# mastbaum/sxmc

Measured on AMD Instinct MI355X. Metric: NLL evals/sec (10^8 samples, 3 obs, 12 signals) + experiments/sec at 1/2/4/8 GPUs, higher is better.
Workload: dtype f64 exact; f32-on-u16-codes filter decides the unambiguous samples

## Files before the change

sxmc_amd/csrc/fill_kernels.inc.h:

```cpp
#pragma once

#include "sxmc_device_types.h"

#pragma clang fp contract(off)

#ifndef SXMC_MEASURE
#define SXMC_MEASURE 0
#endif

namespace sxfill {

__device__ __forceinline__ constexpr unsigned sx_dbg(unsigned dbg_arg) { return SXMC_MEASURE ? dbg_arg : 0u; }

template <int N>
struct IntC {
  static constexpr int value = N;
  constexpr operator int() const { return N; }
};
template <unsigned long... I>
struct ISeq {};
template <int N, unsigned long... I>
struct MakeISeq : MakeISeq<N - 1, (unsigned long)(N - 1), I...> {};
template <unsigned long... I>
struct MakeISeq<0, I...> {
  typedef ISeq<I...> type;
// ... 479 lines not shown
#pragma unroll 4
      for (unsigned b = tid; b < B; b += nthreads) {
        const unsigned c = hist[b];
        if (c != 0u) __hip_atomic_fetch_add(&gbins[b], c, __ATOMIC_RELAXED, __HIP_MEMORY_SCOPE_AGENT);
      }
      if (si + 1u < seg_end) {
        __syncthreads();
        for (unsigned b = tid; b < B; b += nthreads) hist[b] = 0u;
      }
    }
    if (tid == 0) {
      const unsigned c = *s_norm;
      if (c != 0u) __hip_atomic_fetch_add(to_global(d.norm), c, __ATOMIC_RELAXED, __HIP_MEMORY_SCOPE_AGENT);
      *s_norm = 0u;
    }
    __syncthreads();
    lds_clean = true;
  }
}

constexpr int kPreOrdered = kFormOrdered;
constexpr int kPreBoxed = kFormBoxed;
constexpr unsigned kOrdMixed = 0xFFFFFFFEu, kOrdSkip = 0xFFFFFFFFu;
typedef float vfloat2 __attribute__((ext_vector_type(2)));

template <unsigned OPC>
__device__ __forceinline__ void apply_ordered_scalar(double& x, const double* c) {
  constexpr int type = (int)(OPC & 15u);
  static_assert(sx_op_npars(OPC) == 1 && (type == SXMC_SYST_SHIFT || type == SXMC_SYST_SCALE || type == SXMC_SYST_CTSCALE),
                "not a monotone systematic");
  const double pc = 0.0 + c[0] * 1.0;
  if constexpr (type == SXMC_SYST_SHIFT) x = x + pc;
  if constexpr (type == SXMC_SYST_SCALE) x = x * (1 + pc);
  if constexpr (type == SXMC_SYST_CTSCALE) x = 1 + (x - 1) * (1 + pc);
}
template <int ORD, unsigned... OPS, unsigned long... I>
__device__ __forceinline__ void run_ordered_scalar(double& x, const double* c, StaticProg<OPS...>, ISeq<I...>) {
  ([&] {
    if constexpr ((int)((OPS >> 4) & 15u) == ORD) apply_ordered_scalar<OPS>(x, c + sx_prog_cstart<OPS...>((int)I));
  }(), ...);
}
template <int NSLOT, int ORD, bool WANT, unsigned... OPS, unsigned long... I>
__device__ __forceinline__ void run_static_part(double (&f)[NSLOT][SXMC_VEC], const double* c, StaticProg<OPS...>,
                                                ISeq<I...>) {
  ([&] {
    if constexpr (((int)((OPS >> 4) & 15u) == ORD) == WANT) apply_static<NSLOT, OPS>(f, c + sx_prog_cstart<OPS...>((int)I));
// ... 1300 lines not shown
  fin = fin && (__builtin_fabs(xl) < __builtin_inf()) && (__builtin_fabs(xh) < __builtin_inf());
}
template <int BX, int XT, unsigned... OPS, unsigned long... I>
__device__ __forceinline__ void run_box_interval(double& xl, double& xh, double tl, double th, bool& fin, const double* c,
                                                 StaticProg<OPS...>, ISeq<I...>) {
  ([&] {
    if constexpr ((int)((OPS >> 4) & 15u) == BX) apply_box_interval<OPS, XT>(xl, xh, tl, th, fin, c + sx_prog_cstart<OPS...>((int)I));
  }(), ...);
}
template <int BX, int XT, unsigned... OPS>
constexpr bool prog_is_boxable(StaticProg<OPS...>) {
  return (true && ... &&
          (sx_op_npars(OPS) == 1 && (int)((OPS >> 4) & 15u) != XT &&
           ((int)(OPS & 15u) != SXMC_SYST_RESOLUTION_SCALE ||
            ((int)((OPS >> 4) & 15u) == BX && (int)((OPS >> 8) & 15u) == XT))));
}

#ifndef SXMC_BOX_DRAIN
#define SXMC_BOX_DRAIN 2
#endif
#ifndef SXMC_BOX_GQ
#define SXMC_BOX_GQ 0
#endif
#ifndef SXMC_BOX_PREFETCH
#define SXMC_BOX_PREFETCH 0
#endif
template <int NOBS, int NSLOT, typename PROG>
__device__ __forceinline__ void fill_boxed_body(const SxSignalDesc* __restrict__ descs, const SxSegment* __restrict__ segs,
                                                const unsigned* __restrict__ blk_off, unsigned layout, unsigned dbg_arg) {
  const unsigned dbg = sx_dbg(dbg_arg);
  static_assert(!PROG::dynamic && NOBS == 1 && NSLOT == 3, "one streamed observable, one truth field, the boxed observable");
  constexpr int BX = 2, XT = 1;
  static_assert(prog_is_boxable<BX, XT>(PROG{}), "not a program the boxed form can run");
  constexpr int NC = PROG::ncoef > 0 ? PROG::ncoef : 1;
#ifndef SXMC_BOX_RING
#define SXMC_BOX_RING 8
#endif
  constexpr int kRing = SXMC_BOX_RING;
  constexpr int kDrain = SXMC_BOX_DRAIN;
  static_assert(64 % kRing == 0, "a block of 64 units is a whole number of rounds of the ring");
  typedef typename MakeISeq<PROG::n>::type Seq;
  extern __shared__ unsigned lds[];
  const unsigned tid = threadIdx.x;
  const unsigned nthreads = blockDim.x;
  const unsigned lane = tid & (kWave - 1);
  unsigned* s_norm = lds;
// ... 76 lines not shown
      g = g + form[0].a[0] * (d.qbase[0] + 0.5 * d.qstep[0]);
      g = g * sc;
      const double mu = sum_abs * 65536.0 + __builtin_fabs(g) + (double)nbk + 0.25;
      const double epsq = 0.5 * sum_abs * (1.0 + 0x1p-19);
      const double eps = epsq + mu * 0x1p-21 + (form[0].mag + __builtin_fabs(lo)) * sc * 0x1p-44;
      const bool ok = eps < 0.125;
      double e = eps * 1.01, slack = 0x1p-23;
#if SXMC_MEASURE
      {
        const unsigned fr = (dbg >> 8) & 0xFFu, ft = (dbg >> 16) & 0xFFu;
        const double rs = fr ? (double)(fr - 1u) / 64.0 : 1.0, ts = ft ? (double)(ft - 1u) / 64.0 : 1.0;
        e = (epsq + rs * (e - epsq)) * ts;
        slack = slack * rs * ts;
      }
#endif
      af = uniform_f((float)alpha);
      gf = uniform_f((float)(g + e));
      thr = uniform_f((float)(2.0 * e + slack));
      use_q = use_q && (uniform_i(ok ? 1 : 0) != 0);
    }

    unsigned vcnt = 0u;
    unsigned nrow = 0u, ngran = 0u;

    unsigned gword = kOrdSkip, greal = 0u;
    vfloat4 bx_next;
    unsigned pre_next;
    auto meta_load = [&](unsigned it) {
      unsigned vg = vwave32 + (it + lane) * step32;
      vg = vg <= vlast32 ? vg : vlast32;
      bx_next = boxes[vg >> 6];
      pre_next = precol[vg >> 6];
    };
    auto granule_meta = [&](unsigned it) {
      unsigned vg = vwave32 + (it + lane) * step32;
      const bool live = vg <= vlast32;
      vg = live ? vg : vlast32;
      if constexpr (!SXMC_BOX_PREFETCH) meta_load(it);
      const vfloat4 bx = bx_next;
      const unsigned pre = pre_next;
      if constexpr (SXMC_BOX_PREFETCH) meta_load(it + 64u);
      double xl = (double)bx.x, xh = (double)bx.y;
      const double tl = (double)bx.z, th = (double)bx.w;
      bool fin = (__builtin_fabs(xl) < __builtin_inf()) && (__builtin_fabs(xh) < __builtin_inf()) &&
                 (__builtin_fabs(tl) < __builtin_inf()) && (__builtin_fabs(th) < __builtin_inf());
      run_box_interval<BX, XT>(xl, xh, tl, th, fin, craw, PROG{}, Seq{});
      const int i0 = (int)((xl - olo) * osc), i1 = (int)((xh - olo) * osc);
      const int e0 = !(xl >= olo) ? -1 : (!(xl < ohi) ? 0x7FFFFFFF : i0);
      const int e1 = !(xh >= olo) ? -1 : (!(xh < ohi) ? 0x7FFFFFFF : i1);
      const unsigned off = (pre & 0xFFFFFFu) + (unsigned)e0 * (unsigned)ost;
      const unsigned h = fdiv(off, inv_out), rem = off - h * s_out;
      const bool canon = off < (1u << 22) && rem < s_in && (h + 1u) * s_out <= B;
      const bool mixed = !use_q || !fin || e0 != e1 || !canon;
      const bool skip = fin && e0 == e1 && (e0 < 0 || e0 == 0x7FFFFFFF);
      gword = !live ? kOrdSkip : skip ? kOrdSkip : mixed ? kOrdMixed : h * s_in + rem;
      greal = off;
    };

    auto push_granule = [&](unsigned it) {
      if (lane == 0) qgran[2u * ngran] = vwave32 + it * step32;
      ngran += 1u;
    };
    auto push_rows = [&](unsigned rare, unsigned v, unsigned real_off) -> bool {
      unsigned long long mask[SXMC_VEC];
      unsigned total = 0u;
#pragma unroll
      for (int q = 0; q < SXMC_VEC; q++) {
        mask[q] = __builtin_amdgcn_ballot_w64(((rare >> q) & 1u) != 0u);
        total += (unsigned)__builtin_popcountll(mask[q]);
      }
      if (nrow + total > rq_cap) return false;
#pragma unroll
      for (int q = 0; q < SXMC_VEC; q++) {
        if (mask[q] == 0ull) continue;
        const unsigned below = __builtin_amdgcn_mbcnt_hi((unsigned)(mask[q] >> 32),
                                                         __builtin_amdgcn_mbcnt_lo((unsigned)mask[q], 0u));
        if ((rare >> q) & 1u) {
          const unsigned pos = nrow + below;
          qrows[2u * pos] = v * SXMC_VEC + (unsigned)q;
          qrows[2u * pos + 1u] = real_off;
        }
        nrow += (unsigned)__builtin_popcountll(mask[q]);
      }
      return true;
    };

    const int oS4 = (int)(4u * oSp);
    const int oclamp = (dbg & 4u) ? -1 : (int)nbk;
    auto coarse_unit = [&](const vuint2g& w, unsigned it, unsigned v, unsigned word0) {
      int base4 = (int)(4u * (4u + myrep + word0) + 4u * oSp);
      asm volatile("" : "+v"(base4));
      const float c0 = (float)(w.x & 0xFFFFu), c1 = (float)(w.x >> 16), c2 = (float)(w.y & 0xFFFFu), c3 = (float)(w.y >> 16);
      const vfloat2 a2 = {af, af}, g2 = {gf, gf};
      const vfloat2 u01 = __builtin_elementwise_fma(a2, vfloat2{c0, c1}, g2);
      const vfloat2 u23 = __builtin_elementwise_fma(a2, vfloat2{c2, c3}, g2);
      const float us[SXMC_VEC] = {u01.x, u01.y, u23.x, u23.y};
      int addr[SXMC_VEC];
      bool amb[SXMC_VEC];
#pragma unroll
      for (int q = 0; q < SXMC_VEC; q++) {
        const float u = us[q];
        amb[q] = !(__builtin_amdgcn_fractf(u) >= thr);
        int idx;
        asm("v_cvt_flr_i32_f32 %0, %1" : "=v"(idx) : "v"(u));
        int ie;
        asm("v_med3_i32 %0, %1, -1, %2" : "=v"(ie) : "v"(amb[q] ? -1 : idx), "s"(oclamp));
        addr[q] = mad24(ie, oS4, base4);
      }
      const float cmax = __builtin_fmaxf(__builtin_fmaxf(c0, c1), __builtin_fmaxf(c2, c3));
      const bool special = cmax >= (float)SXMC_QCODE_EXACT;
      const bool anyamb = (amb[0] | amb[1]) | (amb[2] | amb[3]);
      if (__builtin_amdgcn_ballot_w64(anyamb || special) != 0ull) {
        const float cs[SXMC_VEC] = {c0, c1, c2, c3};
        unsigned rare = 0u;
#pragma unroll
        for (int q = 0; q < SXMC_VEC; q++) {
          rare |= amb[q] ? (1u << q) : 0u;
          if (cs[q] >= (float)SXMC_QCODE_EXACT) {
            addr[q] = base4 - oS4;
            rare = cs[q] >= (float)SXMC_QCODE_NEVER ? (rare & ~(1u << q)) : (rare | (1u << q));
          }
        }
        const unsigned real_off = (unsigned)__builtin_amdgcn_readlane((int)greal, (int)(it & 63u));
        if (!push_rows(rare, v, real_off)) {
          push_granule(it);
          return;
        }
      }
      if (dbg & 32u) {
        vcnt += (unsigned)(addr[0] ^ addr[1] ^ addr[2] ^ addr[3]) == 12345u ? 1u : 0u;
        return;
      }
#pragma unroll
      for (int q = 0; q < SXMC_VEC; q++) {
        unsigned* wp = reinterpret_cast<unsigned*>(reinterpret_cast<char*>(lds) + addr[q]);
        __hip_atomic_fetch_add(wp, 1u, __ATOMIC_RELAXED, __HIP_MEMORY_SCOPE_WORKGROUP);
      }
    };

    auto count_exact = [&](bool ind, int bin) {
      vcnt += (ind && !((unsigned)bin < B)) ? 1u : 0u;
      if (ind && ((unsigned)bin < B)) {
        __hip_atomic_fetch_add(&hist[myrep + hist_word((unsigned)bin)], 1u, __ATOMIC_RELAXED, __HIP_MEMORY_SCOPE_WORKGROUP);
      }
    };
    auto drain = [&]() {
      if (dbg & 16u) nrow = ngran = 0u;
      vfloat4 rawf[kDrain][NSLOT];
      unsigned prew[kDrain];
      auto load_granule = [&](int s, unsigned g) {
        const unsigned vw = (unsigned)uniform_i((int)qgran[2u * g]);
        const unsigned vc = vw + lane < vlast32 ? vw + lane : vlast32;
#pragma unroll
        for (int k = 0; k < NSLOT; k++) rawf[s][k] = __builtin_nontemporal_load(&col[k][vc]);
        prew[s] = precol[vc >> 6];
      };
      unsigned row = 0u, w1 = 0u;
      float rowf = 0.0f;
// ... 64 lines not shown
      rq[slot] = __builtin_nontemporal_load((gptr<const vuint2g>)((gptr<const char>)qcol + (unsigned long long)o));
      __builtin_amdgcn_sched_barrier(0);
    };
    const unsigned climit = (unsigned)uniform_i((int)oS);
    {
      unsigned it = 0u;
      if constexpr (SXMC_BOX_PREFETCH) meta_load(0u);
#pragma unroll
      for (int i = 0; i < kRing; i++) issue(i, (unsigned)i);
      while (it < niter32) {
        if ((it & 63u) == 0u) granule_meta(it);
        const unsigned block_end = niter32 < (it | 63u) + 1u ? niter32 : (it | 63u) + 1u;
        bool full = false;
        while (it < block_end && !full) {
#pragma unroll
          for (int i = 0; i < kRing; i++) {
#pragma unroll
            for (int e = 0; e < 2; e++) asm volatile("" : "+v"(rq[i][e]));
            const unsigned iu = it + (unsigned)i;
            if (iu < block_end) {
              const unsigned word0 = (unsigned)__builtin_amdgcn_readlane((int)gword, (int)(iu & 63u));
              if (dbg & 1u) {
                vcnt += (rq[i].x == 12345u && word0 == 77u) ? 1u : 0u;
              } else if (word0 < climit) coarse_unit(rq[i], iu, vfirst32 + iu * step32, word0);
              else if (word0 == kOrdMixed) push_granule(iu);
            }
            issue(i, iu + (unsigned)kRing);
          }
          it = block_end - it < (unsigned)kRing ? block_end : it + (unsigned)kRing;
          full = ngran + (unsigned)kRing > gq_drain;
        }
        if (full) {
          drain();
          __builtin_amdgcn_s_waitcnt(0);
        }
      }
    }
    drain();

    {
      unsigned t = vcnt;
#pragma unroll
      for (int off = kWave / 2; off > 0; off >>= 1) t += __shfl_down(t, off, kWave);
      if (lane == 0 && t != 0u) __hip_atomic_fetch_add(&s_norm[0], t, __ATOMIC_RELAXED, __HIP_MEMORY_SCOPE_WORKGROUP);
    }
    __syncthreads();
    {
      gptr<unsigned> gbins = to_global(d.bins);
      const bool more = si + 1u < seg_end;
      const unsigned nwords = nbk * oSp;
      const float invSp = 1.0f / (float)oSp;
      unsigned total = 0u;
#pragma unroll 4
      for (unsigned w = tid; w < nwords; w += nthreads) {
        const unsigned idx = fdiv(w, invSp), r = w - idx * oSp;
        unsigned n = 0u;
        for (unsigned rep = 0; rep < R; rep++) n += hist[rep * rstride + oSp + w];
        if (r < oS) {
          total += n;
          const unsigned h = fdiv(r, inv_in);
          if (n != 0u) {
            __hip_atomic_fetch_add(&gbins[h * s_out + idx * s_in + (r - h * s_in)], n, __ATOMIC_RELAXED, __HIP_MEMORY_SCOPE_AGENT);
          }
        }
      }
#pragma unroll
      for (int off = kWave / 2; off > 0; off >>= 1) total += __shfl_down(total, off, kWave);
      if (lane == 0 && total != 0u) __hip_atomic_fetch_add(&s_norm[0], total, __ATOMIC_RELAXED, __HIP_MEMORY_SCOPE_WORKGROUP);
      __syncthreads();
      if (more) {
        for (unsigned b = 4u * tid; b < cstride; b += 4u * nthreads) {
          *reinterpret_cast<vuint4g*>(&hist[b]) = vuint4g{0u, 0u, 0u, 0u};
        }
      }
      if (tid == 0) {
        const unsigned n = s_norm[0];
        if (n != 0u) __hip_atomic_fetch_add(to_global(d.norm), n, __ATOMIC_RELAXED, __HIP_MEMORY_SCOPE_AGENT);
        s_norm[0] = 0u;
      }
    }
    __syncthreads();
    lds_clean = true;
  }
}

template <int NOBS, int NSLOT, bool LDS_HIST, typename PROG, int PREW>
__global__ __launch_bounds__(1024) void fill_kernel(const SxSignalDesc* __restrict__ descs,
                                                    const SxSegment* __restrict__ segs,
                                                    const unsigned* __restrict__ blk_off, unsigned hist_words,
                                                    unsigned dbg) {
  fill_body<NOBS, NSLOT, LDS_HIST, PROG, PREW>(descs, segs, blk_off, hist_words, dbg);
}

template <int NOBS, int NSLOT, typename PROG>
__global__ __launch_bounds__(1024) void fill_sparse_kernel(const SxSignalDesc* __restrict__ descs,
                                                           const SxSegment* __restrict__ segs,
                                                           const unsigned* __restrict__ blk_off, unsigned smax,
                                                           unsigned dbg) {
  fill_sparse_body<NOBS, NSLOT, PROG>(descs, segs, blk_off, smax, dbg);
}

#ifndef SXMC_ORDERED_BOUND
// ... 22 lines not shown
```

sxmc_amd/csrc/layout_kernels.hip:

```cpp
#include "nll_device.h"
#include "sxmc_host.h"

#include <hipcub/hipcub.hpp>

#include <cmath>
#include <cstring>
#include <limits>

#pragma clang fp contract(off)

namespace {

struct KeyPlan {
  unsigned mask;
  unsigned outside;
  unsigned radix[SXMC_MAX_NFIELDS];
};

__global__ __launch_bounds__(256) void bucket_key_kernel(const SxSignalDesc* __restrict__ dp, KeyPlan plan,
                                                         const unsigned* __restrict__ rows_in,
                                                         unsigned* __restrict__ keys, unsigned* __restrict__ rows) {
  const SxSignalDesc& d = *dp;
  const unsigned long long n = d.nsamples;
  const unsigned long long step = (unsigned long long)gridDim.x * blockDim.x;
// ... 199 lines not shown
                                                             unsigned long long n, unsigned short* __restrict__ qcol,
                                                             unsigned* __restrict__ tally) {
  const unsigned long long step = (unsigned long long)gridDim.x * blockDim.x;
  unsigned nexact = 0u, nnever = 0u;
  for (unsigned long long i = (unsigned long long)blockIdx.x * blockDim.x + threadIdx.x; i < n; i += step) {
    const double x = (double)col[i];
    unsigned code;
    if (!(fabs(x) < __builtin_inf())) {
      code = SXMC_QCODE_NEVER;
      nnever++;
    } else {
      const double t = (x - base) / qstep;
      bool exact = !(t >= 0.0 && t < (double)(SXMC_QCODE_MAX + 1u));
      const unsigned q = exact ? 0u : (unsigned)t;
      const double centre = base + ((double)q + 0.5) * qstep;
      if (!(fabs(x - centre) <= 0.5 * qstep * (1.0 + 0x1p-20))) exact = true;
      code = exact ? SXMC_QCODE_EXACT : q;
      nexact += exact ? 1u : 0u;
    }
    qcol[i] = (unsigned short)code;
  }
  if (nexact) atomicAdd(&tally[0], nexact);
  if (nnever) atomicAdd(&tally[1], nnever);
}

struct SampleGeom {
  int nobs;
  int has_cuts;
  int nbins[3];
  double lower[3], upper[3], width[3];
  double scale[3];
  float bottom[3], top[3];
  float cut_lo[3], cut_hi[3];
};

__device__ __forceinline__ int sample_side(float xf, unsigned idx, double lower, double upper, double scale) {
  const double x = (double)xf;
  if (!(x >= lower)) return -1;
  if (!(x < upper)) return 1;
  const long long j = (long long)((x - lower) * scale);
  return j < (long long)idx ? -1 : j > (long long)idx ? 1 : 0;
}

__device__ __forceinline__ float sample_float(double xd, unsigned idx, const SampleGeom& g, int k) {
  const float x0 = (float)xd;
  float xf = x0;
// ... 194 lines not shown
}

hipError_t sx_column_codes16(const float* col, double base, double step, unsigned long long n, unsigned short* qcol,
                             unsigned long long* tally, hipStream_t s) {
  sxhost::DeviceBuffer<unsigned> tmp;
  hipError_t e = (hipError_t)tmp.alloc(2);
  if (e != hipSuccess) return e;
  unsigned* const d = tmp.get();
  e = hipMemsetAsync(d, 0, sizeof(unsigned) * 2, s);
  if (e == hipSuccess && n) {
    hipLaunchKernelGGL(column_codes16_kernel, dim3(grid_for(n, 16384)), dim3(256), 0, s, col, base, step, n, qcol, d);
    e = hipGetLastError();
  }
  unsigned h[2] = {0u, 0u};
  if (e == hipSuccess) e = hipMemcpyAsync(h, d, sizeof h, hipMemcpyDeviceToHost, s);
  hipError_t e2 = hipStreamSynchronize(s);
  if (tally) {
    tally[0] = h[0];
    tally[1] = h[1];
  }
  return e != hipSuccess ? e : e2;
}

hipError_t sx_hist_cdf(const unsigned* d_bins, unsigned* d_cdf, int nbins_total, hipStream_t s) {
  size_t temp_bytes = 0;
  hipError_t e = hipcub::DeviceScan::InclusiveSum(nullptr, temp_bytes, d_bins, d_cdf, nbins_total, s);
  if (e != hipSuccess) return e;
  sxhost::DeviceBuffer<void> temp;
  e = (hipError_t)temp.alloc(temp_bytes ? temp_bytes : 16);
  if (e != hipSuccess) return e;
  e = hipcub::DeviceScan::InclusiveSum(temp.get(), temp_bytes, d_bins, d_cdf, nbins_total, s);
  hipError_t e2 = hipStreamSynchronize(s);
  return e != hipSuccess ? e : e2;
}

hipError_t sx_inclusive_sum_u32(const unsigned* d_in, unsigned* d_out, int n, void* temp, size_t& temp_bytes,
                                hipStream_t s) {
  return hipcub::DeviceScan::InclusiveSum(temp, temp_bytes, d_in, d_out, n, s);
}

hipError_t sx_random_sample(const unsigned* d_cdf, int nbins_total, int nobs, const int* nbins, const double* lower,
                            const double* upper, const double* scale, const float* cut_lo, const float* cut_hi,
                            unsigned long long seed, unsigned long long n, float dataset, float* d_out,
                            unsigned* d_exhausted, hipStream_t s) {
  if (n == 0) return hipSuccess;
  SampleGeom g{};
// ... 21 lines not shown
```

sxmc_amd/csrc/sxmc_device.h:

```cpp
#pragma once

#include <hip/hip_runtime.h>
#include <stdint.h>

#include <string>

#include "../../include/sxmc_hip.h"

#include "step_end_plan.h"
#include "sxmc_device_types.h"

struct SxStepArgs {
  size_t nsignals, nsources;
  const double* means;
  const double* sigmas;
  sxmc_rng_state* rng;
  double* nll_current;
  double* nll_proposed;
  double* v_current;
  double* v_proposed;
  int* accepted;
  int* counter;
  float* jump_buffer;
  int nparameters;
// ... 124 lines not shown
hipError_t sx_launch_fill(const SxLaunchShape& shape, const SxSignalDesc* d_descs, const SxSegment* d_segs,
                          const unsigned* d_blk_off, hipStream_t s);
hipError_t sx_launch_fill_sparse_runs(const SxLaunchShape& shape, const SxSignalDesc* d_descs, const SxSegment* d_segs,
                                      const unsigned* d_blk_off, hipStream_t s);
bool sx_fill_has_specialization(int nobs, int nslot);
int sx_fill_find_program(int form, int nobs, int nslot, int nops, const unsigned* ops);
bool sx_fill_supports(int prog, int form, int lds_hist, int sparse_runs);
bool sx_fill_weighted_supports(int prog, int lds_hist);
hipError_t sx_launch_prebin(const SxSignalDesc* d_desc, unsigned long long npad, unsigned mask, int width, void* out,
                            hipStream_t s);
hipError_t sx_bucket_keys(const SxSignalDesc* d_desc, unsigned long long nsamples, unsigned mask, const unsigned* radix,
                          unsigned outside, const unsigned* d_rows_in, unsigned* d_keys, unsigned* d_rows,
                          hipStream_t s);
hipError_t sx_order_keys(const float* d_col, unsigned long long nsamples, unsigned* d_keys, unsigned* d_rows,
                         hipStream_t s);
hipError_t sx_bucket_edges(const float* d_col, const unsigned* d_valid, unsigned long long ngranules, float* d_edges,
                           hipStream_t s);
hipError_t sx_box_keys(const float* d_colx, const float* d_colt, unsigned long long nsamples, int pass, int nstrata,
                       const unsigned* bounds, unsigned* d_keys, unsigned* d_rows, hipStream_t s);
hipError_t sx_bucket_boxes(const float* d_colx, const float* d_colt, const unsigned* d_valid, unsigned long long ngranules,
                           float* d_boxes, hipStream_t s);
hipError_t sx_column_codes16(const float* col, double base, double step, unsigned long long n, unsigned short* qcol,
                             unsigned long long* tally, hipStream_t s);
hipError_t sx_bucket_sort(const unsigned* keys_in, unsigned* keys_out, const unsigned* rows_in, unsigned* rows_out,
                          unsigned long long n, int bits, hipStream_t s);
hipError_t sx_bucket_first(const unsigned* sorted_keys, unsigned long long n, unsigned* d_first, hipStream_t s);
hipError_t sx_bucket_gather(const float* cols, unsigned long long pitch, int ncols, const int* col_list,
                            const unsigned* sorted_rows, const unsigned* d_src, const unsigned* d_valid,
                            unsigned long long ngranules, float* out, unsigned long long out_pitch, hipStream_t s);
hipError_t sx_column_minmax(const float* cols, unsigned long long pitch, int ncols, unsigned long long n, float* out,
                            hipStream_t s);
hipError_t sx_column_codes(const float* cols, unsigned long long pitch, int nslots, const double* base, const double* step,
                           unsigned long long n, unsigned* qcol, unsigned long long* tally, hipStream_t s);
hipError_t sx_hist_cdf(const unsigned* d_bins, unsigned* d_cdf, int nbins_total, hipStream_t s);
hipError_t sx_random_sample(const unsigned* d_cdf, int nbins_total, int nobs, const int* nbins, const double* lower,
                            const double* upper, const double* scale, const float* cut_lo, const float* cut_hi,
                            unsigned long long seed, unsigned long long n, float dataset, float* d_out,
                            unsigned* d_exhausted, hipStream_t s);
hipError_t sx_hist_project(const unsigned* d_bins, unsigned long long total, unsigned stride, unsigned nb,
                           unsigned long long* d_out, unsigned max_blocks, hipStream_t s);
hipError_t sx_launch_eval_pdf(const SxSignalDesc* d_descs, int nsig, unsigned long long max_points,
                              hipStream_t s);
template <typename W>
hipError_t sx_launch_eval_nll(const SxSignalDesc* d_descs, int nsig, unsigned long long npoints,
                              const W* weight, const double* pars, const double* nexpected, const unsigned* n_mc,
                              const short* source_id, const unsigned* norms, double* sums,
// ... 91 lines not shown
```

sxmc_amd/csrc/sxmc_group.cpp:

```cpp
#include "sxmc_host.h"

using namespace sxhost;

namespace sxhost {
std::atomic<int> g_stepping_groups{0};

int proposal_factor_check(const double* factor, int nparameters, size_t nsignals) {
  if (factor && (nparameters > 256 || nsignals > 256)) {
    return fail(SXMC_ERR_SHAPE, "a proposal factor needs the staged step end: at most 256 parameters and 256 signals");
  }
  return SXMC_OK;
}

SxStepArgs sx_step_args(const sxmc_step_args& p, size_t nsignals, const double* factor) {
  SxStepArgs a;
  a.factor = factor;
  a.nsignals = nsignals;
  a.nsources = p.nsources;
  a.means = p.d_means;
  a.sigmas = p.d_sigmas;
  a.rng = p.d_rng;
  a.nll_current = p.d_nll_current;
  a.nll_proposed = p.d_nll_proposed;
  a.v_current = p.d_v_current;
// ... 960 lines not shown
}

static void algorithmic_bytes(const sxmc_group* g, const LaunchPlan& plan, double* fill_read, double* hist, double* event) {
  double fr = 0, hb = 0, ev = 0;
  for (size_t i = 0; i < g->members.size(); i++) {
    const sxmc_hist* h = g->members[i];
    const SxSignalDesc& d = g->h_descs[i];
    int pre_w = 0, pre_dims = 0;
    bool codes = false;
    for (const LaunchClass& c : plan.classes) {
      for (int idx : c.member_idx) {
        if (idx == (int)i && c.shape.form != kFormRows) {
          pre_w = sx_form_pre_bytes(c.shape.form);
          for (int k = 0; k < d.nobs; k++) pre_dims += (c.pre_mask >> k) & 1u;
        }
        if (idx == (int)i) codes = c.codes;
      }
    }
    if (const SampleStore::Bucketed* bk = i < plan.member_bucket.size() ? plan.member_bucket[i] : nullptr) {
      const bool ord = bk->sort && bk->sort->ordered >= 0;
      const bool box = ord && bk->sort->box_truth >= 0;
      const double row_bytes = (codes && bk->d_qcol) ? (bk->q16 ? 2.0 : 4.0 * (double)((bk->nq + 1) / 2))
                                                     : 4.0 * (double)(bk->fields.size() - (ord ? 1 : 0));
      fr += (double)bk->nkept * row_bytes + ((box ? 16.0 : ord ? 8.0 : 0.0) + (bk->runs > 1 ? 8.0 : 4.0)) * (double)bk->ngranules;
    } else {
      fr += (double)h->nsamples * (4.0 * (d.nslot - pre_dims) + pre_w + (h->mult ? 4.0 : 0.0));
    }
    if (h->total_nbins <= kLdsMaxBins) {
      hb += 4.0 * (double)h->total_nbins;
    } else if (g->sparse_ready && g->cfg_sparse) {
      hb += 2.0 * 4.0 * (double)std::max(h->ntargets, 1);
    } else {
      hb += 2.0 * 4.0 * (double)h->total_nbins;
    }
    ev += 16.0 * (double)d.npoints;
  }
  *fill_read = fr;
  *hist = hb;
  *event = ev;
}

int sxmc_group_algorithmic_bytes(sxmc_group_t g, double* fill_read, double* hist, double* event) {
  SX_REQUIRE(g && fill_read && hist && event, "null argument");
  int rc = group_refresh(g);
  if (rc) return rc;
  algorithmic_bytes(g, active_plan(g), fill_read, hist, event);
  return SXMC_OK;
// ... 4 lines not shown
```

sxmc_amd/csrc/sxmc_launch_plan.cpp:

```cpp
#include "sxmc_host.h"

using namespace sxhost;

namespace sxhost {

using sxplan::apportion_workgroups;

template <typename T>
hipError_t upload(const std::vector<T>& v, DeviceBuffer<T>& d, size_t room = 0) {
  const hipError_t e = (hipError_t)d.alloc(std::max(v.size(), room));
  return (e != hipSuccess || v.empty()) ? e : hipMemcpy(d.get(), v.data(), sizeof(T) * v.size(), hipMemcpyHostToDevice);
}

void member_slots(const sxmc_hist* h, std::vector<int>& slot_col) {
  slot_col.clear();
  for (int k = 0; k < h->nobs; k++) slot_col.push_back(k);
  std::vector<int> extra;
  for (const HostSyst& s : h->systs) {
    if (s.obs >= h->nobs) extra.push_back(s.obs);
    if (s.type == SXMC_SYST_RESOLUTION_SCALE && s.extra_field >= h->nobs) extra.push_back(s.extra_field);
  }
  std::sort(extra.begin(), extra.end());
  extra.erase(std::unique(extra.begin(), extra.end()), extra.end());
  for (int c : extra) slot_col.push_back(c);
// ... 223 lines not shown
  b->runs = runs;
  b->sort = bs;
  sxplan::BucketedLayout lay;
  sxplan::bucketed_layout(bs->lsrc, bs->lvalid, bs->lwhich, bs->keys, bs->key_pre, bs->nkeys_total, runs, pack_rows, lay);
  const size_t P = lay.P, A = lay.A;
  const std::vector<unsigned>&psrc = lay.psrc, &pvalid = lay.pvalid, &ppre = lay.ppre, &pkp = lay.pkp;
  b->ngranules = P;
  b->nkept = bs->nkept;
  b->pitch = std::max<size_t>(64, P * 256);
  DeviceBuffer<unsigned> dsrc, dvalid;
  SX_BUF(b->d_cols.alloc(b->pitch * fields.size()));
  SX_BUF(b->d_gpre.alloc(A));
  SX_BUF(b->d_gkp.alloc(2 * A));
  SX_HIP(hipMemcpy(b->d_gpre.get(), ppre.data(), sizeof(unsigned) * A, hipMemcpyHostToDevice));
  SX_HIP(hipMemcpy(b->d_gkp.get(), pkp.data(), sizeof(unsigned) * 2 * A, hipMemcpyHostToDevice));
  SX_BUF(dsrc.alloc(A ? A : 4));
  SX_BUF(dvalid.alloc(A ? A : 4));
  SX_HIP(hipMemcpy(dsrc.get(), psrc.data(), A * 4, hipMemcpyHostToDevice));
  SX_HIP(hipMemcpy(dvalid.get(), pvalid.data(), A * 4, hipMemcpyHostToDevice));
  SX_HIP(sx_bucket_gather(st.d_cols.get(), h->pitch, (int)fields.size(), fields.data(), bs->d_rows.get(), dsrc.get(),
                          dvalid.get(), P, b->d_cols.get(), b->pitch, nullptr));
  if (bs->ordered >= 0 && bs->box_truth >= 0) {
    SX_REQUIRE(fields.size() >= 2, "a boxed layout streams its observable and the truth field");
    SX_BUF(b->d_gbox.alloc(4 * A));
    SX_HIP(hipMemset(b->d_gbox.get(), 0xFF, sizeof(float) * 4 * A));
    SX_HIP(sx_bucket_boxes(b->d_cols.get() + (fields.size() - 1) * b->pitch, b->d_cols.get() + (fields.size() - 2) * b->pitch,
                           dvalid.get(), P, b->d_gbox.get(), nullptr));
    {
      std::vector<float> hb(4 * P);
      if (P) SX_HIP(hipMemcpy(hb.data(), b->d_gbox.get(), sizeof(float) * 4 * P, hipMemcpyDeviceToHost));
      std::vector<double> ex, et;
      for (size_t p = 0; p < P; p++) {
        const float x0 = hb[4 * p], x1 = hb[4 * p + 1], t0 = hb[4 * p + 2], t1 = hb[4 * p + 3];
        if (!(std::isfinite(x0) && std::isfinite(x1) && std::isfinite(t0) && std::isfinite(t1))) continue;
        ex.push_back((double)x1 - (double)x0);
        et.push_back((double)t1 - (double)t0);
      }
      auto trimmed = [](std::vector<double>& v) {
        if (v.empty()) return 0.0;
        std::sort(v.begin(), v.end());
        const size_t keep = std::max<size_t>(1, v.size() * 9 / 10);
        double sum = 0;
        for (size_t i = 0; i < keep; i++) sum += v[i];
        return sum / (double)keep;
      };
      b->box_dx = trimmed(ex);
      b->box_dt = trimmed(et);
    }
// ... 37 lines not shown
    b->qbase[m] = cw.base[(size_t)m];
    b->qstep[m] = cw.step[(size_t)m];
  }
  double ambiguous = 0;
  for (int m = 0; m < nq && m < cd.nobs; m++) ambiguous += (double)cd.nbins[m] * cw.step[(size_t)m] / (cd.upper[m] - cd.lower[m]);
  static const bool gate_lifted = [] {
    const char* e = measure_env("SXMC_CODES_GATE");
    return e && e[0] == '1';
  }();
  if (!(ambiguous <= 2e-3) && !gate_lifted) return SXMC_OK;
  if (b->d_qcol.alloc(boxed ? b->pitch / 2 : b->pitch * (size_t)((nq + 1) / 2)) != 0) {
    (void)hipGetLastError();
    return SXMC_OK;
  }
  unsigned long long tally[2] = {0, 0};
  b->q16 = boxed;
  hipError_t e = boxed ? sx_column_codes16(b->d_cols.get(), b->qbase[0], b->qstep[0], n, reinterpret_cast<unsigned short*>(b->d_qcol.get()),
                                           tally, nullptr)
                       : sx_column_codes(b->d_cols.get(), b->pitch, nq, b->qbase, b->qstep, n, b->d_qcol.get(), tally, nullptr);
  if (e != hipSuccess || (double)tally[0] > 0.02 * (double)std::max<size_t>(b->nkept, 1)) {
    b->d_qcol.reset();
    if (e != hipSuccess) return fail(SXMC_ERR_HIP, std::string("codes of a bucketed table: ") + hipGetErrorString(e));
    return SXMC_OK;
  }
  b->nq = nq;
  b->q_exact_rows = tally[0];
  b->q_never_rows = tally[1];
  return SXMC_OK;
}


int build_bucket_tables(sxmc_hist* h, const SampleStore::BucketSort* bs) {
  if (h->btab_valid && h->btab_mask == bs->mask && h->btab_points_version == h->points_version) return SXMC_OK;
  reset_bucket_tables(h);
  sxplan::BucketTables bt;
  sxplan::bucket_tables(bs->nkeys_total, bs->mask, bs->radix, h->nbins.data(), h->stride.data(), h->nobs, h->targets, bt);
  const std::vector<unsigned>&dir = bt.dir, &tkeys = bt.tkeys, &tslot = bt.tslot;
  SX_HIP(upload(dir, h->d_bdir));
  SX_HIP(upload(tkeys, h->d_btkeys, 4));
  SX_HIP(upload(tslot, h->d_btslot, 4));
  h->btab_mask = bs->mask;
  h->btab_points_version = h->points_version;
  h->btab_valid = true;
  return SXMC_OK;
}

// ... 692 lines not shown
```

sxmc_amd/csrc/sxmc_rtc.cpp:

```cpp
#include <hip/hip_runtime.h>
#include <hip/hip_ext.h>
#include <hip/hiprtc.h>

#include <map>
#include <mutex>
#include <string>
#include <vector>

#include "rtc_sources.h"
#include "sxmc_device.h"

namespace {

std::mutex g_mutex;
std::map<std::string, hipFunction_t> g_cache;
std::map<std::string, std::string> g_failed;

std::string join(const char* const* pieces) {
  std::string s;
  for (int i = 0; pieces[i]; i++) s += pieces[i];
  return s;
}

std::string signature(bool chains, int bound, bool dbg = true) {
// ... 29 lines not shown
           ", 1>(one, segs, blk_off, w, dbg);\n}\n";
  }
  if (k.nchain > 1) {
    return s + signature(true, 1024, false) + "  fill_multi_body<" + shape + prog + ", " + std::to_string(k.form) + ", " +
           std::to_string(k.nchain) + ">(chains, segs, blk_off, w);\n}\n";
  }
  if (k.sparse_runs) {
    return s + signature(false, 1024) + "  fill_sparse_body<" + shape + prog + ">(descs, segs, blk_off, w, dbg);\n}\n";
  }
  return s + signature(false, 1024) + "  fill_body<" + shape + (k.lds_hist ? "true" : "false") + ", " + prog + ", " +
         std::to_string(k.form) + ">(descs, segs, blk_off, w, dbg);\n}\n";
}

std::string spec_key(const SxRtcSpec& k) {
  std::string s = std::to_string(k.nobs) + "/" + std::to_string(k.nslot) + "/" + std::to_string(k.lds_hist) + "/" +
                  std::to_string(k.form) + "/" + std::to_string(k.sparse_runs) + "/" + std::to_string(k.nchain) + "/" +
                  std::to_string(k.max_threads) + ":";
  for (int i = 0; i < k.nops; i++) s += std::to_string(k.ops[i]) + ",";
  return s;
}

bool compile(const SxRtcSpec& k, std::vector<char>& code, std::string& err) {
  code.clear();
  const std::string src = kernel_source(k), types = join(kRtcTypesSrc), fill = join(kRtcFillSrc);
  const char* headers[] = {types.c_str(), fill.c_str()};
  const char* names[] = {"sxmc_device_types.h", "fill_kernels.inc.h"};
  hiprtcProgram prog = nullptr;
  hiprtcResult r = hiprtcCreateProgram(&prog, src.c_str(), "sx_rtc_fill.hip", 2, headers, names);
  if (r != HIPRTC_SUCCESS) {
    err = std::string("hiprtcCreateProgram: ") + hiprtcGetErrorString(r);
    return false;
  }
  std::vector<const char*> opts = {"--offload-arch=" SXMC_ARCH, "-O3", "-std=c++17", "-ffp-contract=off", "-fno-fast-math"};
#if defined(SXMC_CACHED_LOADS) && SXMC_CACHED_LOADS
  opts.push_back("-DSXMC_CACHED_LOADS=1");
#endif
#if defined(SXMC_MEASURE) && SXMC_MEASURE
  opts.push_back("-DSXMC_MEASURE=1");
#endif
  r = hiprtcCompileProgram(prog, (int)opts.size(), opts.data());
  if (r != HIPRTC_SUCCESS) {
    size_t n = 0;
    (void)hiprtcGetProgramLogSize(prog, &n);
    std::string log(n, '\0');
    if (n) (void)hiprtcGetProgramLog(prog, &log[0]);
    err = std::string("hiprtcCompileProgram: ") + hiprtcGetErrorString(r) + "\n" + log;
    (void)hiprtcDestroyProgram(&prog);
    return false;
  }
  size_t n = 0;
  r = hiprtcGetCodeSize(prog, &n);
// ... 86 lines not shown
```

Measured before the change: 13940.

## Precompute per-granule code ranges to take a plain fast path in boxed fill

Adds a setup kernel that records each granule's min and max u16 code and a flag for special codes, stored after the box array. The boxed fill kernel checks whether the whole code range maps inside the histogram and, if so, tags the granule as plain. Plain granules skip the bin clamp and the special-code checks. LDS atomics now use direct address-space-3 pointers. The cost is one extra 4-byte metadata load per granule and a second instantiation of the unit code, which may raise register pressure.

```diff
diff --git a/sxmc_amd/csrc/boxed_plain.h b/sxmc_amd/csrc/boxed_plain.h
--- /dev/null
+++ b/sxmc_amd/csrc/boxed_plain.h
@@ -0,0 +1,23 @@
+#pragma once
+
+#include "sxmc_device_types.h"
+
+#if defined(__HIPCC__) || defined(__HIPCC_RTC__)
+#define SX_PLAIN_HD __host__ __device__
+#else
+#define SX_PLAIN_HD
+#endif
+
+constexpr unsigned kBoxRangeFlagged = 0xFFFFu;
+
+SX_PLAIN_HD inline unsigned sx_box_range_word(unsigned cmin, unsigned cmax, bool special, bool none) {
+  if (none) return kBoxRangeFlagged;
+  return (cmax << 16) | (special ? kBoxRangeFlagged : cmin);
+}
+
+SX_PLAIN_HD inline bool sx_box_granule_plain(float af, float gf, unsigned nbins, unsigned range_word) {
+  const unsigned cmin = range_word & 0xFFFFu, cmax = range_word >> 16;
+  const float u0 = __builtin_fmaf(af, (float)cmin, gf), u1 = __builtin_fmaf(af, (float)cmax, gf);
+  const float top = (float)nbins;
+  return (cmin <= SXMC_QCODE_MAX) & (cmin <= cmax) & (u0 >= 0.0f) & (u0 < top) & (u1 >= 0.0f) & (u1 < top);
+}
diff --git a/sxmc_amd/csrc/fill_kernels.inc.h b/sxmc_amd/csrc/fill_kernels.inc.h
--- a/sxmc_amd/csrc/fill_kernels.inc.h
+++ b/sxmc_amd/csrc/fill_kernels.inc.h
@@ -1,6 +1,7 @@
 #pragma once
 
 #include "sxmc_device_types.h"
+#include "boxed_plain.h"
 
 #pragma clang fp contract(off)
 
@@ -526,6 +527,7 @@
 constexpr int kPreOrdered = kFormOrdered;
 constexpr int kPreBoxed = kFormBoxed;
 constexpr unsigned kOrdMixed = 0xFFFFFFFEu, kOrdSkip = 0xFFFFFFFFu;
+constexpr unsigned kBoxPlain = 0x40000000u;
 typedef float vfloat2 __attribute__((ext_vector_type(2)));
 
 template <unsigned OPC>
@@ -1872,6 +1874,9 @@
 #ifndef SXMC_BOX_GQ
 #define SXMC_BOX_GQ 0
 #endif
+#ifndef SXMC_BOX_DSADDR
+#define SXMC_BOX_DSADDR 1
+#endif
 #ifndef SXMC_BOX_PREFETCH
 #define SXMC_BOX_PREFETCH 0
 #endif
@@ -1994,15 +1999,21 @@
 
     unsigned vcnt = 0u;
     unsigned nrow = 0u, ngran = 0u;
+#if SXMC_MEASURE
+    unsigned pad[SXMC_VEC] = {0u, 0u, 0u, 0u};
+    unsigned nrare_units = 0u;
+#endif
 
     unsigned gword = kOrdSkip, greal = 0u;
     vfloat4 bx_next;
-    unsigned pre_next;
+    unsigned pre_next, rng_next;
+    gptr<const unsigned> ranges = (gptr<const unsigned>)boxes + 4ull * (unsigned long long)(d.nvec >> 6);
     auto meta_load = [&](unsigned it) {
       unsigned vg = vwave32 + (it + lane) * step32;
       vg = vg <= vlast32 ? vg : vlast32;
       bx_next = boxes[vg >> 6];
       pre_next = precol[vg >> 6];
+      rng_next = ranges[vg >> 6];
     };
     auto granule_meta = [&](unsigned it) {
       unsigned vg = vwave32 + (it + lane) * step32;
@@ -2010,7 +2021,7 @@
       vg = live ? vg : vlast32;
       if constexpr (!SXMC_BOX_PREFETCH) meta_load(it);
       const vfloat4 bx = bx_next;
-      const unsigned pre = pre_next;
+      const unsigned pre = pre_next, rng = rng_next;
       if constexpr (SXMC_BOX_PREFETCH) meta_load(it + 64u);
       double xl = (double)bx.x, xh = (double)bx.y;
       const double tl = (double)bx.z, th = (double)bx.w;
@@ -2025,7 +2036,8 @@
       const bool canon = off < (1u << 22) && rem < s_in && (h + 1u) * s_out <= B;
       const bool mixed = !use_q || !fin || e0 != e1 || !canon;
       const bool skip = fin && e0 == e1 && (e0 < 0 || e0 == 0x7FFFFFFF);
-      gword = !live ? kOrdSkip : skip ? kOrdSkip : mixed ? kOrdMixed : h * s_in + rem;
+      const bool plain = sx_box_granule_plain(af, gf, nbk, rng) && !(dbg & (4u | 128u));
+      gword = !live ? kOrdSkip : skip ? kOrdSkip : mixed ? kOrdMixed : (h * s_in + rem) | (plain ? kBoxPlain : 0u);
       greal = off;
     };
 
@@ -2058,9 +2070,12 @@
     };
 
     const int oS4 = (int)(4u * oSp);
+    typedef __attribute__((address_space(3))) unsigned lds_word;
+    const unsigned lds_base = SXMC_BOX_DSADDR ? (unsigned)(unsigned long long)(lds_word*)lds : 0u;
     const int oclamp = (dbg & 4u) ? -1 : (int)nbk;
-    auto coarse_unit = [&](const vuint2g& w, unsigned it, unsigned v, unsigned word0) {
-      int base4 = (int)(4u * (4u + myrep + word0) + 4u * oSp);
+    auto coarse_unit = [&](auto plain_c, const vuint2g& w, unsigned it, unsigned v, unsigned word0) {
+      constexpr bool PLAIN = decltype(plain_c)::value != 0;
+      int base4 = (int)(4u * (4u + myrep + word0) + 4u * oSp + lds_base);
       asm volatile("" : "+v"(base4));
       const float c0 = (float)(w.x & 0xFFFFu), c1 = (float)(w.x >> 16), c2 = (float)(w.y & 0xFFFFu), c3 = (float)(w.y >> 16);
       const vfloat2 a2 = {af, af}, g2 = {gf, gf};
@@ -2075,22 +2090,40 @@
         amb[q] = !(__builtin_amdgcn_fractf(u) >= thr);
         int idx;
         asm("v_cvt_flr_i32_f32 %0, %1" : "=v"(idx) : "v"(u));
-        int ie;
-        asm("v_med3_i32 %0, %1, -1, %2" : "=v"(ie) : "v"(amb[q] ? -1 : idx), "s"(oclamp));
+        int ie = amb[q] ? -1 : idx;
+        if constexpr (!PLAIN) asm("v_med3_i32 %0, %1, -1, %2" : "=v"(ie) : "v"(ie), "s"(oclamp));
         addr[q] = mad24(ie, oS4, base4);
       }
-      const float cmax = __builtin_fmaxf(__builtin_fmaxf(c0, c1), __builtin_fmaxf(c2, c3));
-      const bool special = cmax >= (float)SXMC_QCODE_EXACT;
+      bool special = false;
+      if constexpr (!PLAIN) {
+        const float cmax = __builtin_fmaxf(__builtin_fmaxf(c0, c1), __builtin_fmaxf(c2, c3));
+        special = cmax >= (float)SXMC_QCODE_EXACT;
+      }
       const bool anyamb = (amb[0] | amb[1]) | (amb[2] | amb[3]);
+#if SXMC_MEASURE
+      if (dbg & (1u << 28)) {
+#pragma unroll
+        for (int q = 0; q < SXMC_VEC; q++) asm volatile("v_xor_b32 %0, %1, %0" : "+v"(pad[q]) : "v"(w.x));
+      }
+      if (dbg & (1u << 29)) {
+#pragma unroll
+        for (int q = 0; q < SXMC_VEC; q++) asm volatile("v_xor_b32 %0, %1, %0" : "+v"(pad[q]) : "v"(w.y));
+      }
+#endif
       if (__builtin_amdgcn_ballot_w64(anyamb || special) != 0ull) {
+#if SXMC_MEASURE
+        nrare_units += 1u;
+#endif
         const float cs[SXMC_VEC] = {c0, c1, c2, c3};
         unsigned rare = 0u;
 #pragma unroll
         for (int q = 0; q < SXMC_VEC; q++) {
           rare |= amb[q] ? (1u << q) : 0u;
-          if (cs[q] >= (float)SXMC_QCODE_EXACT) {
-            addr[q] = base4 - oS4;
-            rare = cs[q] >= (float)SXMC_QCODE_NEVER ? (rare & ~(1u << q)) : (rare | (1u << q));
+          if constexpr (!PLAIN) {
+            if (cs[q] >= (float)SXMC_QCODE_EXACT) {
+              addr[q] = base4 - oS4;
+              rare = cs[q] >= (float)SXMC_QCODE_NEVER ? (rare & ~(1u << q)) : (rare | (1u << q));
+            }
           }
         }
         const unsigned real_off = (unsigned)__builtin_amdgcn_readlane((int)greal, (int)(it & 63u));
@@ -2105,7 +2138,11 @@
       }
 #pragma unroll
       for (int q = 0; q < SXMC_VEC; q++) {
+#if SXMC_BOX_DSADDR
+        lds_word* wp = (lds_word*)(unsigned long)(unsigned)addr[q];
+#else
         unsigned* wp = reinterpret_cast<unsigned*>(reinterpret_cast<char*>(lds) + addr[q]);
+#endif
         __hip_atomic_fetch_add(wp, 1u, __ATOMIC_RELAXED, __HIP_MEMORY_SCOPE_WORKGROUP);
       }
     };
@@ -2216,7 +2253,8 @@
               const unsigned word0 = (unsigned)__builtin_amdgcn_readlane((int)gword, (int)(iu & 63u));
               if (dbg & 1u) {
                 vcnt += (rq[i].x == 12345u && word0 == 77u) ? 1u : 0u;
-              } else if (word0 < climit) coarse_unit(rq[i], iu, vfirst32 + iu * step32, word0);
+              } else if ((word0 ^ kBoxPlain) < climit) coarse_unit(IntC<1>{}, rq[i], iu, vfirst32 + iu * step32, word0 ^ kBoxPlain);
+              else if (word0 < climit) coarse_unit(IntC<0>{}, rq[i], iu, vfirst32 + iu * step32, word0);
               else if (word0 == kOrdMixed) push_granule(iu);
             }
             issue(i, iu + (unsigned)kRing);
@@ -2234,6 +2272,9 @@
 
     {
       unsigned t = vcnt;
+#if SXMC_MEASURE
+      t += (pad[0] ^ pad[1] ^ pad[2] ^ pad[3]) == 0x9E3779B9u && (dbg & 1u) ? 1u : 0u;
+#endif
 #pragma unroll
       for (int off = kWave / 2; off > 0; off >>= 1) t += __shfl_down(t, off, kWave);
       if (lane == 0 && t != 0u) __hip_atomic_fetch_add(&s_norm[0], t, __ATOMIC_RELAXED, __HIP_MEMORY_SCOPE_WORKGROUP);
@@ -2269,9 +2310,14 @@
       }
       if (tid == 0) {
         const unsigned n = s_norm[0];
-        if (n != 0u) __hip_atomic_fetch_add(to_global(d.norm), n, __ATOMIC_RELAXED, __HIP_MEMORY_SCOPE_AGENT);
+        if (n != 0u && !(dbg & (1u << 30))) __hip_atomic_fetch_add(to_global(d.norm), n, __ATOMIC_RELAXED, __HIP_MEMORY_SCOPE_AGENT);
         s_norm[0] = 0u;
       }
+#if SXMC_MEASURE
+      if ((dbg & (1u << 30)) && lane == 0 && nrare_units != 0u) {
+        __hip_atomic_fetch_add(to_global(d.norm), nrare_units, __ATOMIC_RELAXED, __HIP_MEMORY_SCOPE_AGENT);
+      }
+#endif
     }
     __syncthreads();
     lds_clean = true;
diff --git a/sxmc_amd/csrc/layout_kernels.hip b/sxmc_amd/csrc/layout_kernels.hip
--- a/sxmc_amd/csrc/layout_kernels.hip
+++ b/sxmc_amd/csrc/layout_kernels.hip
@@ -1,3 +1,4 @@
+#include "boxed_plain.h"
 #include "nll_device.h"
 #include "sxmc_host.h"
 
@@ -245,6 +246,32 @@
   }
   if (nexact) atomicAdd(&tally[0], nexact);
   if (nnever) atomicAdd(&tally[1], nnever);
+}
+
+__global__ __launch_bounds__(256) void code_ranges16_kernel(const unsigned short* __restrict__ qcol,
+                                                            unsigned long long ngranules, unsigned* __restrict__ ranges) {
+  const unsigned lane = threadIdx.x & 63u;
+  const unsigned long long wave = ((unsigned long long)blockIdx.x * blockDim.x + threadIdx.x) >> 6;
+  const unsigned long long nwaves = ((unsigned long long)gridDim.x * blockDim.x) >> 6;
+  for (unsigned long long p = wave; p < ngranules; p += nwaves) {
+    unsigned lo = 0xFFFFu, hi = 0u;
+    bool special = false;
+    for (unsigned i = 0; i < 4u; i++) {
+      const unsigned c = qcol[p * 256ull + 4u * lane + i];
+      special = special || c >= SXMC_QCODE_EXACT;
+      if (c < SXMC_QCODE_EXACT) {
+        lo = c < lo ? c : lo;
+        hi = c > hi ? c : hi;
+      }
+    }
+    for (int off = 32; off > 0; off >>= 1) {
+      const unsigned l2 = __shfl_down(lo, off, 64), h2 = __shfl_down(hi, off, 64);
+      lo = l2 < lo ? l2 : lo;
+      hi = h2 > hi ? h2 : hi;
+    }
+    const bool anyspecial = __ballot(special) != 0ull;
+    if (lane == 0) ranges[p] = sx_box_range_word(lo, hi, anyspecial, lo > hi);
+  }
 }
 
 struct SampleGeom {
@@ -485,6 +512,12 @@
   return e != hipSuccess ? e : e2;
 }
 
+hipError_t sx_code_ranges16(const unsigned short* qcol, unsigned long long ngranules, unsigned* d_ranges, hipStream_t s) {
+  if (ngranules == 0) return hipSuccess;
+  hipLaunchKernelGGL(code_ranges16_kernel, dim3(grid_for(ngranules * 64ull, 16384)), dim3(256), 0, s, qcol, ngranules, d_ranges);
+  return hipGetLastError();
+}
+
 hipError_t sx_hist_cdf(const unsigned* d_bins, unsigned* d_cdf, int nbins_total, hipStream_t s) {
   size_t temp_bytes = 0;
   hipError_t e = hipcub::DeviceScan::InclusiveSum(nullptr, temp_bytes, d_bins, d_cdf, nbins_total, s);
diff --git a/sxmc_amd/csrc/sxmc_device.h b/sxmc_amd/csrc/sxmc_device.h
--- a/sxmc_amd/csrc/sxmc_device.h
+++ b/sxmc_amd/csrc/sxmc_device.h
@@ -170,6 +170,7 @@
                            float* d_boxes, hipStream_t s);
 hipError_t sx_column_codes16(const float* col, double base, double step, unsigned long long n, unsigned short* qcol,
                              unsigned long long* tally, hipStream_t s);
+hipError_t sx_code_ranges16(const unsigned short* qcol, unsigned long long ngranules, unsigned* d_ranges, hipStream_t s);
 hipError_t sx_bucket_sort(const unsigned* keys_in, unsigned* keys_out, const unsigned* rows_in, unsigned* rows_out,
                           unsigned long long n, int bits, hipStream_t s);
 hipError_t sx_bucket_first(const unsigned* sorted_keys, unsigned long long n, unsigned* d_first, hipStream_t s);
diff --git a/sxmc_amd/csrc/sxmc_group.cpp b/sxmc_amd/csrc/sxmc_group.cpp
--- a/sxmc_amd/csrc/sxmc_group.cpp
+++ b/sxmc_amd/csrc/sxmc_group.cpp
@@ -1006,7 +1006,7 @@
       const bool box = ord && bk->sort->box_truth >= 0;
       const double row_bytes = (codes && bk->d_qcol) ? (bk->q16 ? 2.0 : 4.0 * (double)((bk->nq + 1) / 2))
                                                      : 4.0 * (double)(bk->fields.size() - (ord ? 1 : 0));
-      fr += (double)bk->nkept * row_bytes + ((box ? 16.0 : ord ? 8.0 : 0.0) + (bk->runs > 1 ? 8.0 : 4.0)) * (double)bk->ngranules;
+      fr += (double)bk->nkept * row_bytes + ((box ? 20.0 : ord ? 8.0 : 0.0) + (bk->runs > 1 ? 8.0 : 4.0)) * (double)bk->ngranules;
     } else {
       fr += (double)h->nsamples * (4.0 * (d.nslot - pre_dims) + pre_w + (h->mult ? 4.0 : 0.0));
     }
diff --git a/sxmc_amd/csrc/sxmc_launch_plan.cpp b/sxmc_amd/csrc/sxmc_launch_plan.cpp
--- a/sxmc_amd/csrc/sxmc_launch_plan.cpp
+++ b/sxmc_amd/csrc/sxmc_launch_plan.cpp
@@ -269,8 +269,8 @@
                           dvalid.get(), P, b->d_cols.get(), b->pitch, nullptr));
   if (bs->ordered >= 0 && bs->box_truth >= 0) {
     SX_REQUIRE(fields.size() >= 2, "a boxed layout streams its observable and the truth field");
-    SX_BUF(b->d_gbox.alloc(4 * A));
-    SX_HIP(hipMemset(b->d_gbox.get(), 0xFF, sizeof(float) * 4 * A));
+    SX_BUF(b->d_gbox.alloc(5 * A));
+    SX_HIP(hipMemset(b->d_gbox.get(), 0xFF, sizeof(float) * 5 * A));
     SX_HIP(sx_bucket_boxes(b->d_cols.get() + (fields.size() - 1) * b->pitch, b->d_cols.get() + (fields.size() - 2) * b->pitch,
                            dvalid.get(), P, b->d_gbox.get(), nullptr));
     {
@@ -354,6 +354,15 @@
     b->d_qcol.reset();
     if (e != hipSuccess) return fail(SXMC_ERR_HIP, std::string("codes of a bucketed table: ") + hipGetErrorString(e));
     return SXMC_OK;
+  }
+  if (boxed) {
+    e = sx_code_ranges16(reinterpret_cast<const unsigned short*>(b->d_qcol.get()), b->ngranules,
+                         reinterpret_cast<unsigned*>(b->d_gbox.get()) + 4 * b->ngranules, nullptr);
+    if (e == hipSuccess) e = hipDeviceSynchronize();
+    if (e != hipSuccess) {
+      b->d_qcol.reset();
+      return fail(SXMC_ERR_HIP, std::string("code ranges of a boxed table: ") + hipGetErrorString(e));
+    }
   }
   b->nq = nq;
   b->q_exact_rows = tally[0];
diff --git a/sxmc_amd/csrc/sxmc_rtc.cpp b/sxmc_amd/csrc/sxmc_rtc.cpp
--- a/sxmc_amd/csrc/sxmc_rtc.cpp
+++ b/sxmc_amd/csrc/sxmc_rtc.cpp
@@ -75,11 +75,11 @@
 
 bool compile(const SxRtcSpec& k, std::vector<char>& code, std::string& err) {
   code.clear();
-  const std::string src = kernel_source(k), types = join(kRtcTypesSrc), fill = join(kRtcFillSrc);
-  const char* headers[] = {types.c_str(), fill.c_str()};
-  const char* names[] = {"sxmc_device_types.h", "fill_kernels.inc.h"};
+  const std::string src = kernel_source(k), types = join(kRtcTypesSrc), fill = join(kRtcFillSrc), plain = join(kRtcPlainSrc);
+  const char* headers[] = {types.c_str(), fill.c_str(), plain.c_str()};
+  const char* names[] = {"sxmc_device_types.h", "fill_kernels.inc.h", "boxed_plain.h"};
   hiprtcProgram prog = nullptr;
-  hiprtcResult r = hiprtcCreateProgram(&prog, src.c_str(), "sx_rtc_fill.hip", 2, headers, names);
+  hiprtcResult r = hiprtcCreateProgram(&prog, src.c_str(), "sx_rtc_fill.hip", 3, headers, names);
   if (r != HIPRTC_SUCCESS) {
     err = std::string("hiprtcCreateProgram: ") + hiprtcGetErrorString(r);
     return false;
```

Result: slower. 13500 (-3.1%).
